# airl-iisc/MRFP

Hardware: AMD Instinct MI355X
Metric: train images/sec (higher is better)
Workload: dtype bf16; 1 GPU; resnet-101 DeepLabV3+ + MRFP+ (HRFP+NP+ on, HRFP re-drawn every step), 768x768, 16 images/GPU, fwd+bwd+SGD, synthetic 19-class, random-init weights; global_batch=16, parallelism=dp1

## Files before the change

include/mrfp_hip.h:

```cpp
#ifndef MRFP_HIP_H
#define MRFP_HIP_H

#include <stdint.h>

#ifdef __cplusplus
extern "C" {
#endif

typedef enum { MRFP_F32 = 0, MRFP_BF16 = 1, MRFP_F16 = 2 } mrfp_dtype;

int mrfp_version(void);
const char* mrfp_last_error(void);

int64_t mrfp_stats_nslab(int64_t B, int64_t Ho);

int mrfp_stats_fwd(const void* x, int dtype, int64_t B, int64_t Ho, int64_t Wo, int64_t C,
                   int64_t Hs, int64_t Ws, const int32_t* tabH, const int32_t* tabW,
                   float* ws, void* stream);

int mrfp_stats_bwd(const void* dy, const void* x, const void* y, const float* mean,
                   const float* fA, const float* fS, int per_image, int dtype, int64_t B, int64_t Ho, int64_t Wo, int64_t C,
                   int64_t Hs, int64_t Ws, const int32_t* tabH, const int32_t* tabW,
                   float* ws, void* stream);
int mrfp_stats_bwd_mask(const void* dy, const void* x, const void* mask, const float* mean, int per_image, int dtype, int64_t B,
// ... 160 lines not shown
                    int dtype, int64_t B, int64_t HW, int64_t C, int64_t ignore_index, int per_image, void* stream);
int mrfp_upsample_region_fwd(const void* P, int64_t ld, const int64_t* target, int dtype, int64_t B, int64_t Hi, int64_t Wi,
                             int64_t H, int64_t W, int64_t C, int64_t ignore_index, const float* weight, int kind, float smooth,
                             int present_only, int per_image, float* ws, float* out, void* stream);
int mrfp_upsample_region_bwd(const void* P, int64_t ld, const int64_t* target, const float* out, const float* gscale,
                             void* dlogits, int64_t Cd, int dtype, int64_t B, int64_t Hi, int64_t Wi, int64_t H, int64_t W,
                             int64_t C, int64_t ignore_index, int per_image, void* stream);

int64_t mrfp_sort_tile_items(void);
int64_t mrfp_sort_scan_sweep(void);
int64_t mrfp_sort_pairs_ws_bytes(int64_t n, int64_t S);
int mrfp_sort_pairs(const void* keys_in, const void* payload_in, void* keys_out, void* payload_out, int64_t n,
                    const int64_t* offsets, int64_t S, int bits, void* ws, void* stream);

int64_t mrfp_lovasz_group_classes(void);
int64_t mrfp_lovasz_ws_bytes(int64_t B, int64_t HW, int64_t C, int per_image);
int64_t mrfp_lovasz_out_floats(int64_t B, int64_t HW, int64_t C, int per_image);
int mrfp_lovasz_fwd(const void* logits, const int64_t* target, int dtype, int64_t B, int64_t HW, int64_t C,
                    int64_t ignore_index, int all_classes, int per_image, void* ws, float* out, void* stream);
int mrfp_lovasz_bwd(const void* logits, const int64_t* target, const float* out, const float* gscale, void* dlogits,
                    int dtype, int64_t B, int64_t HW, int64_t C, int64_t ignore_index, int per_image, void* stream);
int mrfp_upsample_lovasz_fwd(const void* P, int64_t ld, const int64_t* target, int dtype, int64_t B, int64_t Hi, int64_t Wi,
                             int64_t H, int64_t W, int64_t C, int64_t ignore_index, int all_classes, int per_image, void* ws,
                             float* out, void* stream);
int mrfp_upsample_lovasz_bwd(const void* P, int64_t ld, const int64_t* target, const float* out, const float* gscale,
                             void* dlogits, int64_t Cd, int dtype, int64_t B, int64_t Hi, int64_t Wi, int64_t H, int64_t W,
                             int64_t C, int64_t ignore_index, int per_image, void* stream);
int mrfp_lovasz_errors(const void* scores, int64_t ld, const int64_t* target, int dtype, int64_t B, int64_t Hi, int64_t Wi,
                       int64_t H, int64_t W, int64_t C, int64_t ignore_index, float* errors, void* stream);

int mrfp_argmax_hist(const void* logits, const int64_t* target, int dtype, int64_t npix, int64_t C,
                     int64_t* hist, uint8_t* pred, void* stream);

int mrfp_pack_weight(const float* w, void* wf, void* wd, int dtype, int64_t N, int64_t C, int64_t R, int64_t S,
                     int64_t Npad, int64_t Cpad, void* stream);
int mrfp_pack_weights_batched(const void* jobs, const int64_t* prefix, int64_t njobs, int64_t total, int dtype, void* stream);
int mrfp_conv_fwd(const void* x, const void* wpack, const float* bias, void* y, int dtype,
                  int64_t B, int64_t H, int64_t W, int64_t C, int64_t N, int64_t ldy, int64_t R, int64_t S,
                  int64_t Ho, int64_t Wo, int64_t stride, int64_t pad_h, int64_t pad_w, int64_t dil,
                  int64_t sstride, const void* addend, float* colstats, void* stream);
int mrfp_conv_fwd_act(const void* x, const void* wpack, const float* bias, void* y, int dtype,
                      int64_t B, int64_t H, int64_t W, int64_t C, int64_t N, int64_t ldy, int64_t R, int64_t S,
                      int64_t Ho, int64_t Wo, int64_t stride, int64_t pad_h, int64_t pad_w, int64_t dil,
                      int64_t sstride, const void* addend, int act, void* stream);
int mrfp_pack_weight_folded(const float* w, void* wf, const float* conv_bias, const float* bn_weight, const float* bn_bias,
                            const float* running_mean, const float* running_var, float eps, float* bias_out, int dtype,
                            int64_t N, int64_t C, int64_t R, int64_t S, int64_t Npad, int64_t Cpad, void* stream);
int mrfp_pack_weights_folded_batched(const void* jobs, const int64_t* prefix, int64_t njobs, int64_t total, int dtype, void* stream);
int mrfp_conv_stats_layout(int dtype, int64_t B, int64_t H, int64_t W, int64_t C, int64_t N, int64_t ldy, int64_t R, int64_t S,
                           int64_t Ho, int64_t Wo, int64_t stride, int64_t pad_h, int64_t pad_w, int64_t dil, int64_t sstride, int wstats,
                           int64_t* out);
int64_t mrfp_conv_stats_block_rows(int dtype, int64_t B, int64_t H, int64_t W, int64_t C, int64_t N, int64_t R, int64_t S, int64_t Ho,
                                   int64_t Wo, int64_t stride, int64_t pad_h, int64_t pad_w, int64_t dil, int64_t sstride);
int mrfp_conv_single_launch(int64_t B, int64_t image_bytes);
int mrfp_conv_fwd_wstats(const void* x, const void* wpack, const float* bias, void* y, int dtype,
                         int64_t B, int64_t H, int64_t W, int64_t C, int64_t N, int64_t ldy, int64_t R, int64_t S,
                         int64_t Ho, int64_t Wo, int64_t stride, int64_t pad_h, int64_t pad_w, int64_t dil,
                         const uint8_t* rowweight, float* colstats, void* stream);
int mrfp_conv_fwd_gated(const void* x, const void* wpack, const float* bias, void* y, int dtype,
                        int64_t B, int64_t H, int64_t W, int64_t C, int64_t N, int64_t ldy, int64_t R, int64_t S,
                        int64_t Ho, int64_t Wo, int64_t stride, int64_t pad_h, int64_t pad_w, int64_t dil,
                        int64_t sstride, const void* addend, const void* addend_mask, void* stream);
int mrfp_conv_fwd_lowrank(const void* x, const void* wpack, const float* bias, void* y, int dtype,
                          int64_t B, int64_t H, int64_t W, int64_t C, int64_t N, int64_t ldy, int64_t R, int64_t S,
                          int64_t Ho, int64_t Wo, int64_t stride, int64_t pad_h, int64_t pad_w, int64_t dil,
                          int64_t sstride, const void* addend, float* colstats, const void* lr_x, const void* lr_w, int64_t lr_k,
                          void* stream);
int mrfp_conv_lowrank_ok(int dtype, int64_t B, int64_t H, int64_t W, int64_t C, int64_t N, int64_t ldy, int64_t R, int64_t S,
                         int64_t Ho, int64_t Wo, int64_t stride, int64_t pad_h, int64_t pad_w, int64_t dil);
int mrfp_debug_clock_stamps(int family, uint64_t* out, int64_t n);
int64_t mrfp_conv_wgrad_ws_bytes(int64_t M, int64_t N, int64_t Q);
int mrfp_conv_wgrad(const void* x, const void* dy, float* dw, void* ws, int dtype,
                    int64_t B, int64_t H, int64_t W, int64_t C, int64_t Ctrue, int64_t N, int64_t ldn,
                    int64_t R, int64_t S, int64_t Ho, int64_t Wo, int64_t stride, int64_t pad_h, int64_t pad_w,
                    int64_t dil, void* stream);
int64_t mrfp_conv_wgrad_group_max(void);
int64_t mrfp_conv_wgrad_grouped_ws_bytes(int64_t M, int64_t N, int64_t Q, int64_t count);
int mrfp_conv_wgrad_plan(int dtype, int64_t B, int64_t H, int64_t W, int64_t C, int64_t N, int64_t ldn, int64_t R, int64_t S, int64_t Ho,
                         int64_t Wo, int64_t stride, int64_t pad_h, int64_t pad_w, int64_t dil, int64_t count, int64_t* out);
int mrfp_conv_wgrad_grouped(const void* const* xs, const void* const* dys, float* const* dws, int64_t count, void* ws, int dtype,
                            int64_t B, int64_t H, int64_t W, int64_t C, int64_t Ctrue, int64_t N, int64_t ldn,
                            int64_t R, int64_t S, int64_t Ho, int64_t Wo, int64_t stride, int64_t pad_h, int64_t pad_w,
                            int64_t dil, void* stream);
int mrfp_nchw_to_nhwc_pad(const float* x, void* y, int dtype, int64_t B, int64_t C, int64_t H, int64_t W,
                          int64_t Cpad, void* stream);

int mrfp_sgd_step(float* p, const float* g, float* m, int64_t n, float lr, float momentum,
                  float weight_decay, float gscale, int first, void* stream);

int mrfp_grad_accumulate(float* acc, const float* g, int64_t n, int first, void* stream);

int64_t mrfp_grad_check_nblocks(int64_t n);
int mrfp_grad_check(const float* g, int64_t n, float gscale, void* ws, void* state, int dynamic, float growth,
                    float backoff, int growth_interval, float max_norm, void* stream);
int mrfp_sgd_step_checked(float* p, const float* g, float* m, int64_t n, float lr, float momentum,
                          float weight_decay, const void* state, void* stream);

int mrfp_sgd_step_avg(float* p, const float* g, float* m, float* e, int64_t n, float lr, float momentum,
                      float weight_decay, float gscale, int first, int kind, double decay, int warmup, int start,
                      int every, int t, void* stream);
int mrfp_sgd_step_checked_avg(float* p, const float* g, float* m, float* e, int64_t n, float lr, float momentum,
                              float weight_decay, const void* state, int taken_base, int kind, double decay, int warmup,
                              int start, int every, void* stream);
int mrfp_arena_swap(float* a, float* b, int64_t n, void* stream);

int64_t mrfp_group_moments_ws_bytes(int64_t B, int64_t HW, int64_t C);
// ... 82 lines not shown
```

mrfp_amd/csrc/conv_c64.hip:

```cpp
#include "conv_common.hpp"

namespace mrfp {


struct C64P {
    const char* x;
    const char* w;
    char* y;
    const float* bias;
    const char* addend;
    float* colstats;
    const unsigned char* rowweight;
    int B, H, W, N, ldy, dil;
    int strips;
    int units;
    int spi;
    unsigned xbytes, wbytes, ybytes;
    const char* lr_x;
    const char* lr_w;
    unsigned lrbytes;
};

constexpr int kC64Slots = 4;

template <typename T, int CB, int NCG, bool STATS, bool ADD, int ACT = 0, bool LR = false>
__global__ __launch_bounds__(256, (CB == 1 ? 2 : 1)) void conv3x3_c64_kernel(C64P p) {
    static_assert(!LR || (!STATS && !ADD && ACT == 0), "the low-rank operand excludes statistics, an addend and an activation");
    constexpr int PSN = 4 / NCG;
    constexpr int SW = 64 * PSN;
    constexpr int NPIECE = (SW + 4 + 7) / 8;
    constexpr int NPC = CB * NPIECE;
    constexpr int PWV = (NPC + 3) / 4;
    constexpr int SLOT = NPC * 1024;
    constexpr int KS = 18 * CB;
    constexpr int PIXB = 128 * CB;
    constexpr int ST = 4;
    extern __shared__ __attribute__((aligned(16))) char smem[];
    const int t = threadIdx.x, lane = t & 63;
    const int wave = __builtin_amdgcn_readfirstlane(t >> 6);
    const int l15 = lane & 15, lq = lane >> 4;
    const int cg = wave % NCG, ps = wave / NCG;
    const int n0 = (int)blockIdx.y * 128 + cg * 32, nl = n0 + 8 * lq;
    const int d = p.dil;
    const unsigned lds0 = (unsigned)(size_t)(__attribute__((address_space(3))) char*)smem;
    const i32x4 xw = rsrc_words(p.x, p.xbytes);
    const __amdgpu_buffer_rsrc_t wr = __builtin_amdgcn_make_buffer_rsrc((void*)p.w, 0, (int)p.wbytes, 0x00020000);
    const __amdgpu_buffer_rsrc_t yr = __builtin_amdgcn_make_buffer_rsrc((void*)p.y, 0, (int)p.ybytes, 0x00020000);
    const __amdgpu_buffer_rsrc_t ar = __builtin_amdgcn_make_buffer_rsrc((void*)(p.addend ? p.addend : p.y), 0, (int)p.ybytes, 0x00020000);

    uint4 fw[KS][2];
#pragma unroll
    for (int ks = 0; ks < KS; ++ks)
#pragma unroll
        for (int j = 0; j < 2; ++j) {
            const int n = n0 + 8 * (l15 >> 2) + 4 * j + (l15 & 3);
            fw[ks][j] = bload(wr, n < p.N ? (unsigned)n * (unsigned)(1152 * CB) + (unsigned)(ks * 64 + lq * 16) : kOOB);
        }
#pragma unroll
    for (int ks = 0; ks < KS; ++ks)
#pragma unroll
        for (int j = 0; j < 2; ++j) settle(fw[ks][j]);
    const __amdgpu_buffer_rsrc_t lxr = __builtin_amdgcn_make_buffer_rsrc((void*)p.lr_x, 0, (int)p.lrbytes, 0x00020000);
    uint4 fl[2];
    if constexpr (LR) {
        const __amdgpu_buffer_rsrc_t lwr = __builtin_amdgcn_make_buffer_rsrc((void*)p.lr_w, 0, p.N * 64, 0x00020000);
#pragma unroll
        for (int j = 0; j < 2; ++j) {
            const int n = n0 + 8 * (l15 >> 2) + 4 * j + (l15 & 3);
            fl[j] = bload(lwr, n < p.N ? (unsigned)(n * 64 + lq * 16) : kOOB);
        }
#pragma unroll
        for (int j = 0; j < 2; ++j) settle(fl[j]);
    }
    float bv[2][4];
#pragma unroll
    for (int j = 0; j < 2; ++j)
#pragma unroll
        for (int e = 0; e < 4; ++e) bv[j][e] = (p.bias && nl + 4 * j + e < p.N) ? p.bias[nl + 4 * j + e] : 0.f;

    unsigned foff[3][2];
#pragma unroll
    for (int s = 0; s < 3; ++s) {
        const int px = ps * 64 + l15 + s * d;
#pragma unroll
        for (int kk = 0; kk < 2; ++kk) foff[s][kk] = (unsigned)(px * 128 + ((((kk * 4 + lq) ^ px) & 7) << 4));
    }

    float cs[8], cq[8];
#pragma unroll
    for (int u = 0; u < 8; ++u) { cs[u] = 0.f; cq[u] = 0.f; }

    const long long G = gridDim.x;
    int u = (int)((long long)blockIdx.x * p.units / G);
    const int u1 = (int)((long long)(blockIdx.x + 1) * p.units / G);
    const int Hc0 = (p.H + d - 1) / d;
    const int upi = p.strips * p.H;
    int cur_b = -1;
    auto flush = [&](int b) {
        const long long lo = (long long)b * upi, hi = lo + upi;
        int wf = (int)(lo * G / p.units);
        while ((long long)(wf + 1) * p.units / G <= lo) ++wf;
        while (wf > 0 && (long long)wf * p.units / G > lo) --wf;
        const int slot = (int)blockIdx.x - wf;
        float* out = p.colstats + ((size_t)(b * PSN + ps) * p.spi + slot) * 2 * p.ldy;
#pragma unroll
        for (int k = 0; k < 8; ++k) {
            cs[k] = row16_sum(cs[k]);
            cq[k] = row16_sum(cq[k]);
        }
        if (l15 == 0 && nl < p.N) {
#pragma unroll
            for (int k = 0; k < 8; ++k) {
                out[nl + k] = cs[k];
                out[p.ldy + nl + k] = cq[k];
            }
            if ((long long)u1 >= hi) {
                for (int z = slot + 1; z < p.spi; ++z) {
                    float* oz = p.colstats + ((size_t)(b * PSN + ps) * p.spi + z) * 2 * p.ldy;
#pragma unroll
                    for (int k = 0; k < 8; ++k) {
                        oz[nl + k] = 0.f;
                        oz[p.ldy + nl + k] = 0.f;
                    }
                }
            }
        }
#pragma unroll
        for (int k = 0; k < 8; ++k) { cs[k] = 0.f; cq[k] = 0.f; }
    };
    while (u < u1) {
        const int blk_id = u / p.H, tt = u - blk_id * p.H;
        const int b = blk_id / p.strips, strip = blk_id - b * p.strips;
        const int q = (d == 2 && tt >= Hc0) ? 1 : 0;
        const int i0 = tt - q * Hc0;
        const int Hc = q ? p.H - Hc0 : Hc0;
        int i1 = i0 + (u1 - u);
        if (i1 > Hc) i1 = Hc;
        const int ow0 = strip * SW;
        if constexpr (STATS) {
            if (b != cur_b) {
                if (cur_b >= 0) flush(cur_b);
                cur_b = b;
            }
        }
        const unsigned imgbase = (unsigned)b * (unsigned)p.H * (unsigned)p.W * (unsigned)PIXB;
        const int col0 = ow0 - d + (lane >> 3);
        auto issue_row = [&](int i) {
            const int ih = q + d * i;
            const bool rok = i >= 0 && ih < p.H;
            const unsigned rbase = imgbase + (unsigned)(rok ? ih : 0) * (unsigned)p.W * (unsigned)PIXB;
            const unsigned sbase = lds0 + (unsigned)(((i + 4) & 3) * SLOT);
#pragma unroll
            for (int j = 0; j < PWV; ++j) {
                const int pi = j * 4 + wave;
                if (pi >= NPC) continue;
                const int hf = pi / NPIECE, pp = pi - hf * NPIECE;
                const int col = col0 + 8 * pp, px = 8 * pp + (lane >> 3);
                const bool cok = col >= 0 && col < p.W;
                const unsigned cb = (unsigned)(col * PIXB + hf * 128 + (((lane & 7) ^ (px & 7)) << 4));
                dma16_async(xw, sbase + (unsigned)(pi * 1024), (rok && cok) ? rbase + cb : kOOB);
            }
        };
        issue_row(i0 - 1);
        issue_row(i0);
        issue_row(i0 + 1);
        for (int i = i0; i < i1; ++i) {
            if (i == i0) dma_wait<0>();
            else dma_wait<ST>();
            __builtin_amdgcn_s_barrier();
            if (i + 1 < i1) issue_row(i + 2);
            const int oh = q + d * i;
            uint4 av[4];
            unsigned wt[4];
            const int owl = ow0 + ps * 64 + l15;
            const unsigned ml = (unsigned)((b * p.H + oh) * p.W + owl);
            auto out_off = [&](int bk) {
                return (owl + bk * 16 < p.W && nl < p.N) ? ((ml + (unsigned)(bk * 16)) * (unsigned)p.ldy + (unsigned)nl) * 2u : kOOB;
            };
#pragma unroll
            for (int bk = 0; bk < 4; ++bk) {
                if constexpr (ADD) av[bk] = bload(ar, out_off(bk));
                if constexpr (LR) av[bk] = bload(lxr, owl + bk * 16 < p.W ? (ml + (unsigned)(bk * 16)) * 64u + (unsigned)(lq * 16) : kOOB);
                if constexpr (STATS) {
                    const bool ok = owl + bk * 16 < p.W;
                    wt[bk] = ok ? (p.rowweight ? (unsigned)p.rowweight[ml + bk * 16] : 1u) : 0u;
                }
            }
            f32x4 acc[4][2];
            const unsigned sb[3] = {lds0 + (unsigned)(((i + 3) & 3) * SLOT), lds0 + (unsigned)((i & 3) * SLOT),
                                    lds0 + (unsigned)(((i + 1) & 3) * SLOT)};
            uint4 fx[2][4];
            auto read_x = [&](int ks, uint4 (&f)[4]) {
                const int r = ks / (6 * CB), s = (ks / (2 * CB)) % 3, hf = (ks >> 1) % CB, kk = ks & 1;
                const char* base = smem + (sb[r] - lds0) + hf * (NPIECE * 1024) + foff[s][kk];
#pragma unroll
                for (int bk = 0; bk < 4; ++bk) f[bk] = *reinterpret_cast<const uint4*>(base + bk * 2048);
            };
            read_x(0, fx[0]);
#pragma unroll
            for (int ks = 0; ks < KS; ++ks) {
                if (ks + 1 < KS) read_x(ks + 1, fx[(ks + 1) & 1]);
                __builtin_amdgcn_sched_barrier(0);
#pragma unroll
                for (int bk = 0; bk < 4; ++bk)
#pragma unroll
                    for (int j = 0; j < 2; ++j) {
                        if (ks == 0) {
                            const f32x4 z = {bv[j][0], bv[j][1], bv[j][2], bv[j][3]};
                            acc[bk][j] = z;
                        }
                        Mma16<T>::run(acc[bk][j], fw[ks][j], fx[ks & 1][bk]);
                    }
                __builtin_amdgcn_sched_barrier(0);
            }
            if constexpr (LR) {
#pragma unroll
                for (int bk = 0; bk < 4; ++bk) {
                    f32x4 t0 = {0.f, 0.f, 0.f, 0.f}, t1 = {0.f, 0.f, 0.f, 0.f};
                    Mma16<T>::run(t0, fl[0], av[bk]);
                    Mma16<T>::run(t1, fl[1], av[bk]);
                    av[bk] = make_uint4(pack2<T>(t0[0], t0[1]), pack2<T>(t0[2], t0[3]), pack2<T>(t1[0], t1[1]), pack2<T>(t1[2], t1[3]));
                }
            }
#pragma unroll
            for (int bk = 0; bk < 4; ++bk) {
                uint4 v;
                if constexpr (ADD || LR) {
                    float a[8];
                    unpack2<T>(av[bk].x, a[0], a[1]);
                    unpack2<T>(av[bk].y, a[2], a[3]);
                    unpack2<T>(av[bk].z, a[4], a[5]);
                    unpack2<T>(av[bk].w, a[6], a[7]);
                    v.x = pack2<T>(act_f<ACT>(acc[bk][0][0] + a[0]), act_f<ACT>(acc[bk][0][1] + a[1]));
                    v.y = pack2<T>(act_f<ACT>(acc[bk][0][2] + a[2]), act_f<ACT>(acc[bk][0][3] + a[3]));
                    v.z = pack2<T>(act_f<ACT>(acc[bk][1][0] + a[4]), act_f<ACT>(acc[bk][1][1] + a[5]));
                    v.w = pack2<T>(act_f<ACT>(acc[bk][1][2] + a[6]), act_f<ACT>(acc[bk][1][3] + a[7]));
                } else {
                    v.x = pack2<T>(act_f<ACT>(acc[bk][0][0]), act_f<ACT>(acc[bk][0][1]));
                    v.y = pack2<T>(act_f<ACT>(acc[bk][0][2]), act_f<ACT>(acc[bk][0][3]));
                    v.z = pack2<T>(act_f<ACT>(acc[bk][1][0]), act_f<ACT>(acc[bk][1][1]));
                    v.w = pack2<T>(act_f<ACT>(acc[bk][1][2]), act_f<ACT>(acc[bk][1][3]));
                }
                if constexpr (STATS) {
                    float f[8];
                    unpack2<T>(v.x, f[0], f[1]);
                    unpack2<T>(v.y, f[2], f[3]);
                    unpack2<T>(v.z, f[4], f[5]);
                    unpack2<T>(v.w, f[6], f[7]);
                    const float wb = (float)wt[bk];
#pragma unroll
                    for (int k = 0; k < 8; ++k) {
                        const float wf = f[k] * wb;
                        cs[k] += wf;
                        cq[k] += wf * f[k];
                    }
                }
                u32x4 dv;
                dv.x = v.x; dv.y = v.y; dv.z = v.z; dv.w = v.w;
                __builtin_amdgcn_raw_buffer_store_b128(dv, yr, (int)out_off(bk), 0, 0);
            }
        }
        u += i1 - i0;
        asm volatile("s_waitcnt lgkmcnt(0)" ::: "memory");
        __builtin_amdgcn_s_barrier();
    }
    if constexpr (STATS) {
        if (cur_b >= 0) flush(cur_b);
    }
}

static bool c64_applicable(const ConvP& p, int esz) {
    static const int on = env_switch("MRFP_CONV_C64", 1);
    if (!on || esz != 2) return false;
    if (p.R != 3 || p.S != 3 || p.stride != 1 || p.sstride != 1 || p.Ho != p.H || p.Wo != p.W) return false;
    if (p.dil < 1 || p.dil > 2 || p.pad_h != p.dil || p.pad_w != p.dil) return false;
    if ((p.ldy & 7) != 0) return false;
    if (p.C == 64) { if (p.N != 64 && p.N != 128) return false; }
    else if (p.C == 128) {
        static const int c128 = env_switch("MRFP_CONV_C128", 1);
        if (!c128 || (p.N != 64 && p.N != 128 && p.N != 256)) return false;
        const int SW = p.N == 64 ? 128 : 64;
        if (c128 < 2 && (int64_t)p.B * ((p.W + SW - 1) / SW) * p.H < 32 * kGrid1PerCU) return false;
    } else return false;
    if (p.addend_mask || (p.colstats && p.addend)) return false;
    if ((int64_t)p.M * p.ldy * esz >= (int64_t)kOOB || p.H < 2 * p.dil) return false;
    return true;
}
bool c64_plan(const ConvP& p, int esz, ConvPlan& plan) {
    if (!c64_applicable(p, esz)) return false;
    const int SW = p.N == 64 ? 128 : 64;
    const int64_t upi = (int64_t)((p.W + SW - 1) / SW) * p.H, units = upi * p.B;
    const int64_t cap = p.C == 64 ? kGrid2PerCU : kGrid1PerCU;
    plan.kind = ConvKernel::c64;
    plan.tile_rows = 0;
    plan.grid = (int)(units < cap ? units : cap);
    plan.spi = (int)(upi / (units / plan.grid) + 2);
    const int64_t rows_per_image = (int64_t)(p.N == 64 ? 2 : 1) * plan.spi;
    plan.stats_blocks = p.B * rows_per_image;
    plan.stats_block_rows = -rows_per_image;
    return true;
}

template <typename T, int CB, int NCG, bool STATS, bool ADD, int ACT = 0, bool LR = false>
static int c64_launch(const C64P& q, int grid, hipStream_t st) {
    constexpr int SW = 64 * (4 / NCG), NPIECE = (SW + 4 + 7) / 8;
    const int lds = kC64Slots * CB * NPIECE * 1024 + 1024;
    static bool attr_set = false;
    if (!attr_set) {
        (void)hipFuncSetAttribute(reinterpret_cast<const void*>(&conv3x3_c64_kernel<T, CB, NCG, STATS, ADD, ACT, LR>),
                                  hipFuncAttributeMaxDynamicSharedMemorySize, lds);
        attr_set = true;
    }
    hipLaunchKernelGGL((conv3x3_c64_kernel<T, CB, NCG, STATS, ADD, ACT, LR>), dim3((unsigned)grid, (unsigned)((q.N + 127) / 128)), dim3(256), lds, st, q);
    MRFP_LAUNCH_CHECK();
    return 0;
}
template <typename T, int CB, int NCG>
static int c64_pick(const ConvP& p, const C64P& q, int grid, hipStream_t st, int act) {
    if (q.lr_x) {
        MRFP_CHECK(act == 0 && !p.colstats && !p.addend, "conv_fwd_lowrank: no activation, statistics or addend beside the low-rank operand");
        return c64_launch<T, CB, NCG, false, false, 0, true>(q, grid, st);
    }
    if (act != 0) {
        if (p.colstats) return -1;
        if (act == 1) return p.addend ? c64_launch<T, CB, NCG, false, true, 1>(q, grid, st) : c64_launch<T, CB, NCG, false, false, 1>(q, grid, st);
        return p.addend ? c64_launch<T, CB, NCG, false, true, 2>(q, grid, st) : c64_launch<T, CB, NCG, false, false, 2>(q, grid, st);
    }
    if (p.colstats) return c64_launch<T, CB, NCG, true, false>(q, grid, st);
    if (p.addend) return c64_launch<T, CB, NCG, false, true>(q, grid, st);
    return c64_launch<T, CB, NCG, false, false>(q, grid, st);
}

template <typename T>
static int c64_run_t(const ConvP& p, const ConvPlan& plan, hipStream_t st, int act, const void* lr_x, const void* lr_w) {
    C64P q;
    q.lr_x = (const char*)lr_x; q.lr_w = (const char*)lr_w; q.lrbytes = lr_x ? (unsigned)((int64_t)p.M * 64) : 0u;
    q.x = p.x; q.w = p.w; q.y = p.y; q.bias = p.bias; q.addend = p.addend; q.colstats = p.colstats; q.rowweight = p.rowweight;
    q.B = p.B; q.H = p.H; q.W = p.W; q.N = p.N; q.ldy = p.ldy; q.dil = p.dil;
    const int SW = p.N == 64 ? 128 : 64;
    q.strips = (p.W + SW - 1) / SW;
    q.units = p.B * q.strips * p.H;
    q.spi = plan.spi;
    q.xbytes = p.xbytes; q.wbytes = p.wbytes; q.ybytes = (unsigned)((int64_t)p.M * p.ldy * 2);
    const int grid = plan.grid;
    if (p.C == 64) return p.N == 64 ? c64_pick<T, 1, 2>(p, q, grid, st, act) : c64_pick<T, 1, 4>(p, q, grid, st, act);
    return p.N == 64 ? c64_pick<T, 2, 2>(p, q, grid, st, act) : c64_pick<T, 2, 4>(p, q, grid, st, act);
}
int c64_run(const ConvP& p, const ConvPlan& plan, bool is_f16, hipStream_t st, int act, const void* lr_x, const void* lr_w) {
    MRFP_CHECK(!lr_x == !lr_w, "conv_fwd_lowrank: both low-rank operands or neither");
    return is_f16 ? c64_run_t<f16>(p, plan, st, act, lr_x, lr_w) : c64_run_t<bf16>(p, plan, st, act, lr_x, lr_w);
}

}
```

mrfp_amd/csrc/conv_common.hpp:

```cpp
#pragma once
#include "common.hpp"
#include <stdlib.h>

#ifndef MRFP_VMCNT0
#define MRFP_VMCNT0 0
#endif

#ifndef MRFP_CLOCK_STAMP
#define MRFP_CLOCK_STAMP 0
#endif

namespace mrfp {

constexpr int kGrid1PerCU = kCUs;
constexpr int kGrid2PerCU = 2 * kCUs;

constexpr int kStampSlots = 4096;
#if MRFP_CLOCK_STAMP
struct ClockStamp {
    unsigned long long t0, r0;
    __device__ __forceinline__ void begin() {
        t0 = __builtin_amdgcn_s_memtime();
        r0 = __builtin_amdgcn_s_memrealtime();
        __builtin_amdgcn_s_waitcnt(0xC07F);
// ... 189 lines not shown
    unsigned short h;
    __builtin_memcpy(&h, &x, 2);
    const unsigned sh = (u & 1) ? 16u : 0u, mask = ~(0xffffu << sh), bits = (unsigned)h << sh;
    if ((u >> 1) == 0) v.x = (v.x & mask) | bits;
    else if ((u >> 1) == 1) v.y = (v.y & mask) | bits;
    else if ((u >> 1) == 2) v.z = (v.z & mask) | bits;
    else v.w = (v.w & mask) | bits;
}
template <typename T> __device__ __forceinline__ uint4 chunk_add(const uint4& a, const uint4& b) {
    uint4 r = make_uint4(0u, 0u, 0u, 0u);
#pragma unroll
    for (int u = 0; u < 16 / (int)sizeof(T); ++u) chunk_set<T>(r, u, from_f<T>(to_f(chunk_get<T>(a, u)) + to_f(chunk_get<T>(b, u))));
    return r;
}

template <typename T, int ACT> __device__ __forceinline__ uint4 chunk_act(const uint4& a) {
    uint4 r = make_uint4(0u, 0u, 0u, 0u);
#pragma unroll
    for (int u = 0; u < 16 / (int)sizeof(T); ++u) chunk_set<T>(r, u, from_f<T>(act_f<ACT>(to_f(chunk_get<T>(a, u)))));
    return r;
}

#ifndef MRFP_RR_HOLD
#define MRFP_RR_HOLD 1
#endif
__device__ __forceinline__ uint4 gate_chunk16(const uint4& v, unsigned bits) {
    auto w = [&](unsigned word, int u) {
        const unsigned keep = (((bits >> u) & 1u) ? 0x0000ffffu : 0u) | (((bits >> (u + 1)) & 1u) ? 0xffff0000u : 0u);
        return word & keep;
    };
    return make_uint4(w(v.x, 0), w(v.y, 2), w(v.z, 4), w(v.w, 6));
}

#ifndef MRFP_EARLY_FULL
#define MRFP_EARLY_FULL 1
#endif

enum class ConvKernel { pw, pwk, c64, rr384, rr192, t256x64, t192x128, t96x128, t128x128 };
struct ConvPlan {
    ConvKernel kind;
    int tile_rows;
    int64_t stats_blocks;
    int64_t stats_block_rows;
    int grid, spi;
};

bool pw_plan(const ConvP& p, int esz, ConvPlan& plan);
int pw_run(const ConvP& p, bool is_f16, hipStream_t st, int act = 0);

bool pwk_plan(const ConvP& p, int esz, ConvPlan& plan);
int pwk_run(const ConvP& p, bool is_f16, hipStream_t st, int act = 0);

bool c64_plan(const ConvP& p, int esz, ConvPlan& plan);
int c64_run(const ConvP& p, const ConvPlan& plan, bool is_f16, hipStream_t st, int act = 0, const void* lr_x = nullptr,
            const void* lr_w = nullptr);

constexpr int kWgMaxGroup = 32;
struct WgGroup {
    const char* x[kWgMaxGroup];
    const char* dy[kWgMaxGroup];
};
inline WgGroup make_wg_group(const void* const* xs, const void* const* dys, int64_t count) {
    WgGroup g;
    for (int i = 0; i < kWgMaxGroup; ++i) {
        g.x[i] = (const char*)xs[i < count ? i : 0];
        g.dy[i] = (const char*)dys[i < count ? i : 0];
    }
    return g;
}

struct ClassWalk {
    int Wp, a, L, R, Wr, splits;
};
inline bool class_walk(int64_t ncls, int64_t U, int per_round, int64_t count, ClassWalk& w) {
    w.Wp = (int)(per_round / count);
    if (ncls * U < w.Wp) w.Wp = (int)(ncls * U);
    w.a = (int)(w.Wp / ncls);
    if (w.a < 1) return false;
    w.L = (int)((ncls * U + w.Wp - 1) / w.Wp);
    const int64_t main = (int64_t)w.a * w.L < U ? (int64_t)w.a * w.L : U;
    w.R = (int)(U - main);
    w.Wr = (int)(w.Wp - w.a * ncls);
    if (w.R > 0 && w.Wr == 0) return false;
    w.splits = w.a + (w.R > 0 ? 2 : 0);
    return true;
}
inline int64_t class_walk_slots(int64_t ncls, int per_round, int64_t count) {
    const int64_t a = (per_round / count) / ncls;
    return a < 1 ? 0 : a + 2;
}
struct WgradGeom {
    int esz;
    int64_t B, H, W, C, N, ldn, R, S, Ho, Wo, stride, pad_h, pad_w, dil, count;
    int64_t M() const { return B * Ho * Wo; }
    int64_t Q() const { return R * S * C; }
    bool pointwise() const { return R == 1 && S == 1 && stride == 1 && pad_h == 0 && pad_w == 0 && H == Ho && W == Wo; }
};
enum class WgradKernel { wg3, wg1, t64x256, t128x128, t256x128 };
enum { kWgDma = 1, kWgDense = 2 };
struct WgradPlan {
    WgradKernel kind;
    int variant;
    int splits;
    int klen;
    int grid;
    int tiles;
// ... 15 lines not shown
```

mrfp_amd/csrc/conv_igemm.hip:

```cpp
#include "conv_common.hpp"
#include <type_traits>

namespace mrfp {

MRFP_STAMP_DECL(g_stamps_igemm)
int stamps_igemm(unsigned long long* out, int n) { return MRFP_STAMP_READ(g_stamps_igemm, out, n); }

template <typename T, int WM, int WN, bool ALIGNED, bool STRIDED, int TM, int TN, bool RR = false, int ACT = 0>
__global__ __launch_bounds__(64 * WM * WN, ((RR && TM * TN >= 6) ? 2 : 3)) void conv_igemm_kernel(ConvP p) {
    constexpr int NT = 64 * WM * WN, BM = 32 * TM * WM, BN = 32 * TN * WN;
    constexpr int SA = BM * 8 / NT, SB = BN * 8 / NT, RSTEP = NT / 8;
    extern __shared__ __attribute__((aligned(16))) char smem[];
    char* const sA0 = smem;
    char* const sB0 = smem + BM * 128;
    MRFP_STAMP_BEGIN();

    const int t = threadIdx.x, lane = t & 63, wave = t >> 6;
    const int wm = wave / WN, wn = wave % WN;
    const int ntn = (p.N + BN - 1) / BN;
    const int tile = xcd_remap(blockIdx.x, gridDim.x);
    const int m0 = (tile / ntn) * BM, n0 = (tile % ntn) * BN;
    const int rbase = t >> 3;
    const int chunk = (t & 7) ^ ((rbase >> 1) & 7);
    const int wrow = __builtin_amdgcn_readfirstlane(wave) * 8;
// ... 757 lines not shown

int mrfp_conv_fwd_gated(const void* x, const void* wpack, const float* bias, void* y, int dtype, int64_t B, int64_t H,
                        int64_t W, int64_t C, int64_t N, int64_t ldy, int64_t R, int64_t S, int64_t Ho, int64_t Wo,
                        int64_t stride, int64_t pad_h, int64_t pad_w, int64_t dil, int64_t sstride, const void* addend,
                        const void* addend_mask, void* stream) {
    MRFP_CHECK(addend && addend_mask, "conv_fwd_gated: addend and its gate mask are required");
    return conv_fwd_impl(x, wpack, bias, y, dtype, B, H, W, C, N, ldy, R, S, Ho, Wo, stride, pad_h, pad_w, dil, sstride, addend,
                         nullptr, stream, addend_mask);
}

int mrfp_conv_fwd_lowrank(const void* x, const void* wpack, const float* bias, void* y, int dtype, int64_t B, int64_t H,
                          int64_t W, int64_t C, int64_t N, int64_t ldy, int64_t R, int64_t S, int64_t Ho, int64_t Wo,
                          int64_t stride, int64_t pad_h, int64_t pad_w, int64_t dil, int64_t sstride, const void* addend,
                          float* colstats, const void* lr_x, const void* lr_w, int64_t lr_k, void* stream) {
    MRFP_CHECK(!addend && !colstats, "conv_fwd_lowrank: the low-rank operand excludes an addend and statistics");
    MRFP_CHECK(lr_x && lr_w && aligned16(lr_x) && aligned16(lr_w), "conv_fwd_lowrank: both low-rank operands are required, 16-byte aligned");
    MRFP_CHECK(lr_k == 32, "conv_fwd_lowrank: the low-rank K is 32, got %lld", (long long)lr_k);
    MRFP_CHECK(dtype == MRFP_BF16 || dtype == MRFP_F16, "conv_fwd_lowrank: 16-bit activations only (dtype %d)", dtype);
    return conv_fwd_impl(x, wpack, bias, y, dtype, B, H, W, C, N, ldy, R, S, Ho, Wo, stride, pad_h, pad_w, dil, sstride, nullptr,
                         nullptr, stream, nullptr, nullptr, 0, lr_x, lr_w);
}

int mrfp_conv_lowrank_ok(int dtype, int64_t B, int64_t H, int64_t W, int64_t C, int64_t N, int64_t ldy, int64_t R, int64_t S,
                         int64_t Ho, int64_t Wo, int64_t stride, int64_t pad_h, int64_t pad_w, int64_t dil) {
    if (!dtype_known(dtype) || dtype_bytes(dtype) != 2) return 0;
    ConvP p;
    if (conv_params(p, dtype, B, H, W, C, N, ldy, R, S, Ho, Wo, stride, pad_h, pad_w, dil, 1, nullptr, nullptr, nullptr, nullptr, nullptr))
        return 0;
    if (!mrfp_conv_single_launch(B, H * W * C * 2)) return 0;
    return conv_plan(p, 2).kind == ConvKernel::c64 ? 1 : 0;
}

int mrfp_conv_stats_layout(int dtype, int64_t B, int64_t H, int64_t W, int64_t C, int64_t N, int64_t ldy, int64_t R, int64_t S,
                           int64_t Ho, int64_t Wo, int64_t stride, int64_t pad_h, int64_t pad_w, int64_t dil, int64_t sstride, int wstats,
                           int64_t* out) {
    MRFP_CHECK(out, "conv_stats_layout: no output array");
    float stats_present;
    unsigned char rows_present;
    ConvP p;
    const int bad = conv_params(p, dtype, B, H, W, C, N, ldy, R, S, Ho, Wo, stride, pad_h, pad_w, dil, sstride, nullptr, nullptr,
                                nullptr, &stats_present, wstats ? &rows_present : nullptr);
    if (bad) return bad;
    const ConvPlan plan = conv_plan(p, dtype_bytes(dtype));
    const int64_t nblk = plan.stats_blocks;
    const bool compact = nblk > kCompactAbove;
    out[0] = nblk;
    out[1] = plan.stats_block_rows;
    out[2] = compact ? nblk + kStatGroups : nblk;
    out[3] = compact ? nblk : 0;
    out[4] = compact ? kStatGroups : nblk;
    return 0;
}

int64_t mrfp_conv_stats_block_rows(int dtype, int64_t B, int64_t H, int64_t W, int64_t C, int64_t N, int64_t R, int64_t S, int64_t Ho,
                                   int64_t Wo, int64_t stride, int64_t pad_h, int64_t pad_w, int64_t dil, int64_t sstride) {
    int64_t lay[5];
    return mrfp_conv_stats_layout(dtype, B, H, W, C, N, N, R, S, Ho, Wo, stride, pad_h, pad_w, dil, sstride, 0, lay) ? 0 : lay[1];
}


}
```

Baseline: 305.8 images/sec.

## Specialize c64 conv row loop by valid column blocks and cost-balance work split

For the CB==2 c64 3x3 conv kernel, the per-row compute body moves into an included header and is instantiated for 0-4 valid 16-column blocks. Partial edge strips then skip MFMA, LDS reads and stores for out-of-range columns. The work split across workgroups is weighted by per-unit cost, with edge strips cheaper, so blocks stay balanced, and the stats-slot lookup is updated to match. A debug API exposes the span layout. Risks are more code variants, register and compile cost, and DMA wait counts now tied to NB.

After: 302.4 images/sec. -1.1%, worse.

```diff
diff --git a/include/mrfp_hip.h b/include/mrfp_hip.h
--- a/include/mrfp_hip.h
+++ b/include/mrfp_hip.h
@@ -236,6 +236,7 @@
                            int64_t* out);
 int64_t mrfp_conv_stats_block_rows(int dtype, int64_t B, int64_t H, int64_t W, int64_t C, int64_t N, int64_t R, int64_t S, int64_t Ho,
                                    int64_t Wo, int64_t stride, int64_t pad_h, int64_t pad_w, int64_t dil, int64_t sstride);
+int64_t mrfp_conv_c64_spans(int dtype, int64_t B, int64_t H, int64_t W, int64_t C, int64_t N, int64_t dil, int64_t* out, int64_t n);
 int mrfp_conv_single_launch(int64_t B, int64_t image_bytes);
 int mrfp_conv_fwd_wstats(const void* x, const void* wpack, const float* bias, void* y, int dtype,
                          int64_t B, int64_t H, int64_t W, int64_t C, int64_t N, int64_t ldy, int64_t R, int64_t S,
diff --git a/mrfp_amd/csrc/conv_c64.hip b/mrfp_amd/csrc/conv_c64.hip
--- a/mrfp_amd/csrc/conv_c64.hip
+++ b/mrfp_amd/csrc/conv_c64.hip
@@ -19,9 +19,45 @@
     const char* lr_x;
     const char* lr_w;
     unsigned lrbytes;
+    int cl;
+    int bycost;
 };
 
 constexpr int kC64Slots = 4;
+
+#ifndef MRFP_C64_EDGES
+#define MRFP_C64_EDGES 1
+#endif
+constexpr bool kC64Edges(int CB) { return MRFP_C64_EDGES && CB == 2; }
+
+struct C64Split {
+    int B, H, strips, units, cl, bycost;
+    long long G;
+    __host__ __device__ long long upi() const { return (long long)strips * H; }
+    __host__ __device__ long long image_cost() const { return (long long)H * (4 * (strips - 1) + cl); }
+    __host__ __device__ int start(long long g) const {
+        if (!bycost) return (int)(g * units / G);
+        const long long CI = image_cost(), T = g * (CI * B) / G, b = T / CI, r = T - b * CI, full = 4LL * (strips - 1) * H;
+        if (b >= B) return units;
+        return (int)(b * upi() + (r < full ? (r + 2) / 4 : (long long)(strips - 1) * H + (r - full + cl / 2) / cl));
+    }
+    __host__ __device__ int first_wg(int b) const {
+        const long long lo = (long long)b * upi();
+        int wf = (int)((long long)b * G / B);
+        while (start(wf + 1) <= lo) ++wf;
+        while (wf > 0 && start(wf) > lo) --wf;
+        return wf;
+    }
+};
+static C64Split c64_split(int B, int H, int W, int C, int N, long long G) {
+    C64Split s;
+    const int SW = N == 64 ? 128 : 64;
+    s.B = B; s.H = H; s.strips = (W + SW - 1) / SW; s.units = B * s.strips * H; s.G = G;
+    const int last = (W - (s.strips - 1) * SW + 15) / 16;
+    s.cl = kC64Edges(C / 64) ? (last < 4 ? last : 4) : 4;
+    s.bycost = s.cl < 4 && s.strips > 1 && s.image_cost() * B / G >= 4;
+    return s;
+}
 
 template <typename T, int CB, int NCG, bool STATS, bool ADD, int ACT = 0, bool LR = false>
 __global__ __launch_bounds__(256, (CB == 1 ? 2 : 1)) void conv3x3_c64_kernel(C64P p) {
@@ -34,7 +70,6 @@
     constexpr int SLOT = NPC * 1024;
     constexpr int KS = 18 * CB;
     constexpr int PIXB = 128 * CB;
-    constexpr int ST = 4;
     extern __shared__ __attribute__((aligned(16))) char smem[];
     const int t = threadIdx.x, lane = t & 63;
     const int wave = __builtin_amdgcn_readfirstlane(t >> 6);
@@ -91,16 +126,22 @@
     for (int u = 0; u < 8; ++u) { cs[u] = 0.f; cq[u] = 0.f; }
 
     const long long G = gridDim.x;
-    int u = (int)((long long)blockIdx.x * p.units / G);
-    const int u1 = (int)((long long)(blockIdx.x + 1) * p.units / G);
+    C64Split sp;
+    sp.B = p.B; sp.H = p.H; sp.strips = p.strips; sp.units = p.units; sp.cl = p.cl; sp.bycost = p.bycost; sp.G = G;
+    int u = kC64Edges(CB) ? sp.start(blockIdx.x) : (int)((long long)blockIdx.x * p.units / G);
+    const int u1 = kC64Edges(CB) ? sp.start((long long)blockIdx.x + 1) : (int)((long long)(blockIdx.x + 1) * p.units / G);
     const int Hc0 = (p.H + d - 1) / d;
     const int upi = p.strips * p.H;
     int cur_b = -1;
     auto flush = [&](int b) {
         const long long lo = (long long)b * upi, hi = lo + upi;
-        int wf = (int)(lo * G / p.units);
-        while ((long long)(wf + 1) * p.units / G <= lo) ++wf;
-        while (wf > 0 && (long long)wf * p.units / G > lo) --wf;
+        int wf;
+        if constexpr (kC64Edges(CB)) wf = sp.first_wg(b);
+        else {
+            wf = (int)(lo * G / p.units);
+            while ((long long)(wf + 1) * p.units / G <= lo) ++wf;
+            while (wf > 0 && (long long)wf * p.units / G > lo) --wf;
+        }
         const int slot = (int)blockIdx.x - wf;
         float* out = p.colstats + ((size_t)(b * PSN + ps) * p.spi + slot) * 2 * p.ldy;
 #pragma unroll
@@ -164,102 +205,33 @@
         issue_row(i0 - 1);
         issue_row(i0);
         issue_row(i0 + 1);
-        for (int i = i0; i < i1; ++i) {
-            if (i == i0) dma_wait<0>();
-            else dma_wait<ST>();
-            __builtin_amdgcn_s_barrier();
-            if (i + 1 < i1) issue_row(i + 2);
-            const int oh = q + d * i;
-            uint4 av[4];
-            unsigned wt[4];
-            const int owl = ow0 + ps * 64 + l15;
-            const unsigned ml = (unsigned)((b * p.H + oh) * p.W + owl);
-            auto out_off = [&](int bk) {
-                return (owl + bk * 16 < p.W && nl < p.N) ? ((ml + (unsigned)(bk * 16)) * (unsigned)p.ldy + (unsigned)nl) * 2u : kOOB;
-            };
-#pragma unroll
-            for (int bk = 0; bk < 4; ++bk) {
-                if constexpr (ADD) av[bk] = bload(ar, out_off(bk));
-                if constexpr (LR) av[bk] = bload(lxr, owl + bk * 16 < p.W ? (ml + (unsigned)(bk * 16)) * 64u + (unsigned)(lq * 16) : kOOB);
-                if constexpr (STATS) {
-                    const bool ok = owl + bk * 16 < p.W;
-                    wt[bk] = ok ? (p.rowweight ? (unsigned)p.rowweight[ml + bk * 16] : 1u) : 0u;
+#define C64_ROWS(nb) { constexpr int NB = nb, NBA = NB ? NB : 1; (void)NBA;
+        if constexpr (kC64Edges(CB)) {
+            int nb = (p.W - ow0 - ps * 64 + 15) >> 4;
+            nb = nb < 0 ? 0 : nb > 4 ? 4 : nb;
+            switch (nb) {
+            case 4: C64_ROWS(4)
+#include "conv_c64_rows.hpp"
+                } break;
+            case 3: C64_ROWS(3)
+#include "conv_c64_rows.hpp"
+                } break;
+            case 2: C64_ROWS(2)
+#include "conv_c64_rows.hpp"
+                } break;
+            case 1: C64_ROWS(1)
+#include "conv_c64_rows.hpp"
+                } break;
+            default:
+                if constexpr (PSN > 1) C64_ROWS(0)
+#include "conv_c64_rows.hpp"
                 }
-            }
-            f32x4 acc[4][2];
-            const unsigned sb[3] = {lds0 + (unsigned)(((i + 3) & 3) * SLOT), lds0 + (unsigned)((i & 3) * SLOT),
-                                    lds0 + (unsigned)(((i + 1) & 3) * SLOT)};
-            uint4 fx[2][4];
-            auto read_x = [&](int ks, uint4 (&f)[4]) {
-                const int r = ks / (6 * CB), s = (ks / (2 * CB)) % 3, hf = (ks >> 1) % CB, kk = ks & 1;
-                const char* base = smem + (sb[r] - lds0) + hf * (NPIECE * 1024) + foff[s][kk];
-#pragma unroll
-                for (int bk = 0; bk < 4; ++bk) f[bk] = *reinterpret_cast<const uint4*>(base + bk * 2048);
-            };
-            read_x(0, fx[0]);
-#pragma unroll
-            for (int ks = 0; ks < KS; ++ks) {
-                if (ks + 1 < KS) read_x(ks + 1, fx[(ks + 1) & 1]);
-                __builtin_amdgcn_sched_barrier(0);
-#pragma unroll
-                for (int bk = 0; bk < 4; ++bk)
-#pragma unroll
-                    for (int j = 0; j < 2; ++j) {
-                        if (ks == 0) {
-                            const f32x4 z = {bv[j][0], bv[j][1], bv[j][2], bv[j][3]};
-                            acc[bk][j] = z;
-                        }
-                        Mma16<T>::run(acc[bk][j], fw[ks][j], fx[ks & 1][bk]);
-                    }
-                __builtin_amdgcn_sched_barrier(0);
-            }
-            if constexpr (LR) {
-#pragma unroll
-                for (int bk = 0; bk < 4; ++bk) {
-                    f32x4 t0 = {0.f, 0.f, 0.f, 0.f}, t1 = {0.f, 0.f, 0.f, 0.f};
-                    Mma16<T>::run(t0, fl[0], av[bk]);
-                    Mma16<T>::run(t1, fl[1], av[bk]);
-                    av[bk] = make_uint4(pack2<T>(t0[0], t0[1]), pack2<T>(t0[2], t0[3]), pack2<T>(t1[0], t1[1]), pack2<T>(t1[2], t1[3]));
-                }
-            }
-#pragma unroll
-            for (int bk = 0; bk < 4; ++bk) {
-                uint4 v;
-                if constexpr (ADD || LR) {
-                    float a[8];
-                    unpack2<T>(av[bk].x, a[0], a[1]);
-                    unpack2<T>(av[bk].y, a[2], a[3]);
-                    unpack2<T>(av[bk].z, a[4], a[5]);
-                    unpack2<T>(av[bk].w, a[6], a[7]);
-                    v.x = pack2<T>(act_f<ACT>(acc[bk][0][0] + a[0]), act_f<ACT>(acc[bk][0][1] + a[1]));
-                    v.y = pack2<T>(act_f<ACT>(acc[bk][0][2] + a[2]), act_f<ACT>(acc[bk][0][3] + a[3]));
-                    v.z = pack2<T>(act_f<ACT>(acc[bk][1][0] + a[4]), act_f<ACT>(acc[bk][1][1] + a[5]));
-                    v.w = pack2<T>(act_f<ACT>(acc[bk][1][2] + a[6]), act_f<ACT>(acc[bk][1][3] + a[7]));
-                } else {
-                    v.x = pack2<T>(act_f<ACT>(acc[bk][0][0]), act_f<ACT>(acc[bk][0][1]));
-                    v.y = pack2<T>(act_f<ACT>(acc[bk][0][2]), act_f<ACT>(acc[bk][0][3]));
-                    v.z = pack2<T>(act_f<ACT>(acc[bk][1][0]), act_f<ACT>(acc[bk][1][1]));
-                    v.w = pack2<T>(act_f<ACT>(acc[bk][1][2]), act_f<ACT>(acc[bk][1][3]));
-                }
-                if constexpr (STATS) {
-                    float f[8];
-                    unpack2<T>(v.x, f[0], f[1]);
-                    unpack2<T>(v.y, f[2], f[3]);
-                    unpack2<T>(v.z, f[4], f[5]);
-                    unpack2<T>(v.w, f[6], f[7]);
-                    const float wb = (float)wt[bk];
-#pragma unroll
-                    for (int k = 0; k < 8; ++k) {
-                        const float wf = f[k] * wb;
-                        cs[k] += wf;
-                        cq[k] += wf * f[k];
-                    }
-                }
-                u32x4 dv;
-                dv.x = v.x; dv.y = v.y; dv.z = v.z; dv.w = v.w;
-                __builtin_amdgcn_raw_buffer_store_b128(dv, yr, (int)out_off(bk), 0, 0);
-            }
-        }
+                break;
+            }
+        } else C64_ROWS(4)
+#include "conv_c64_rows.hpp"
+        }
+#undef C64_ROWS
         u += i1 - i0;
         asm volatile("s_waitcnt lgkmcnt(0)" ::: "memory");
         __builtin_amdgcn_s_barrier();
@@ -301,6 +273,17 @@
     return true;
 }
 
+int64_t c64_spans(const ConvP& p, const ConvPlan& plan, int64_t* out, int64_t n) {
+    const C64Split sp = c64_split(p.B, p.H, p.W, p.C, p.N, plan.grid);
+    const int64_t G = plan.grid, need = 6 + G + p.B;
+    if (!out) return G;
+    if (n < need) return -need;
+    out[0] = sp.units; out[1] = sp.upi(); out[2] = plan.spi; out[3] = sp.cl; out[4] = sp.bycost;
+    for (int64_t g = 0; g <= G; ++g) out[5 + g] = sp.start(g);
+    for (int b = 0; b < p.B; ++b) out[6 + G + b] = sp.first_wg(b);
+    return G;
+}
+
 template <typename T, int CB, int NCG, bool STATS, bool ADD, int ACT = 0, bool LR = false>
 static int c64_launch(const C64P& q, int grid, hipStream_t st) {
     constexpr int SW = 64 * (4 / NCG), NPIECE = (SW + 4 + 7) / 8;
@@ -341,6 +324,8 @@
     q.strips = (p.W + SW - 1) / SW;
     q.units = p.B * q.strips * p.H;
     q.spi = plan.spi;
+    const C64Split sp = c64_split(p.B, p.H, p.W, p.C, p.N, plan.grid);
+    q.cl = sp.cl; q.bycost = sp.bycost;
     q.xbytes = p.xbytes; q.wbytes = p.wbytes; q.ybytes = (unsigned)((int64_t)p.M * p.ldy * 2);
     const int grid = plan.grid;
     if (p.C == 64) return p.N == 64 ? c64_pick<T, 1, 2>(p, q, grid, st, act) : c64_pick<T, 1, 4>(p, q, grid, st, act);
diff --git a/mrfp_amd/csrc/conv_c64_rows.hpp b/mrfp_amd/csrc/conv_c64_rows.hpp
--- /dev/null
+++ b/mrfp_amd/csrc/conv_c64_rows.hpp
@@ -0,0 +1,97 @@
+        for (int i = i0; i < i1; ++i) {
+            if (i == i0) dma_wait<0>();
+            else dma_wait<NB>();
+            __builtin_amdgcn_s_barrier();
+            if (i + 1 < i1) issue_row(i + 2);
+            if constexpr (NB == 0) continue;
+            const int oh = q + d * i;
+            uint4 av[NBA];
+            unsigned wt[NBA];
+            const int owl = ow0 + ps * 64 + l15;
+            const unsigned ml = (unsigned)((b * p.H + oh) * p.W + owl);
+            auto out_off = [&](int bk) {
+                return (owl + bk * 16 < p.W && nl < p.N) ? ((ml + (unsigned)(bk * 16)) * (unsigned)p.ldy + (unsigned)nl) * 2u : kOOB;
+            };
+#pragma unroll
+            for (int bk = 0; bk < NB; ++bk) {
+                if constexpr (ADD) av[bk] = bload(ar, out_off(bk));
+                if constexpr (LR) av[bk] = bload(lxr, owl + bk * 16 < p.W ? (ml + (unsigned)(bk * 16)) * 64u + (unsigned)(lq * 16) : kOOB);
+                if constexpr (STATS) {
+                    const bool ok = owl + bk * 16 < p.W;
+                    wt[bk] = ok ? (p.rowweight ? (unsigned)p.rowweight[ml + bk * 16] : 1u) : 0u;
+                }
+            }
+            f32x4 acc[NBA][2];
+            const unsigned sb[3] = {lds0 + (unsigned)(((i + 3) & 3) * SLOT), lds0 + (unsigned)((i & 3) * SLOT),
+                                    lds0 + (unsigned)(((i + 1) & 3) * SLOT)};
+            uint4 fx[2][NBA];
+            auto read_x = [&](int ks, uint4 (&f)[NBA]) {
+                const int r = ks / (6 * CB), s = (ks / (2 * CB)) % 3, hf = (ks >> 1) % CB, kk = ks & 1;
+                const char* base = smem + (sb[r] - lds0) + hf * (NPIECE * 1024) + foff[s][kk];
+#pragma unroll
+                for (int bk = 0; bk < NB; ++bk) f[bk] = *reinterpret_cast<const uint4*>(base + bk * 2048);
+            };
+            read_x(0, fx[0]);
+#pragma unroll
+            for (int ks = 0; ks < KS; ++ks) {
+                if (ks + 1 < KS) read_x(ks + 1, fx[(ks + 1) & 1]);
+                __builtin_amdgcn_sched_barrier(0);
+#pragma unroll
+                for (int bk = 0; bk < NB; ++bk)
+#pragma unroll
+                    for (int j = 0; j < 2; ++j) {
+                        if (ks == 0) {
+                            const f32x4 z = {bv[j][0], bv[j][1], bv[j][2], bv[j][3]};
+                            acc[bk][j] = z;
+                        }
+                        Mma16<T>::run(acc[bk][j], fw[ks][j], fx[ks & 1][bk]);
+                    }
+                __builtin_amdgcn_sched_barrier(0);
+            }
+            if constexpr (LR) {
+#pragma unroll
+                for (int bk = 0; bk < NB; ++bk) {
+                    f32x4 t0 = {0.f, 0.f, 0.f, 0.f}, t1 = {0.f, 0.f, 0.f, 0.f};
+                    Mma16<T>::run(t0, fl[0], av[bk]);
+                    Mma16<T>::run(t1, fl[1], av[bk]);
+                    av[bk] = make_uint4(pack2<T>(t0[0], t0[1]), pack2<T>(t0[2], t0[3]), pack2<T>(t1[0], t1[1]), pack2<T>(t1[2], t1[3]));
+                }
+            }
+#pragma unroll
+            for (int bk = 0; bk < NB; ++bk) {
+                uint4 v;
+                if constexpr (ADD || LR) {
+                    float a[8];
+                    unpack2<T>(av[bk].x, a[0], a[1]);
+                    unpack2<T>(av[bk].y, a[2], a[3]);
+                    unpack2<T>(av[bk].z, a[4], a[5]);
+                    unpack2<T>(av[bk].w, a[6], a[7]);
+                    v.x = pack2<T>(act_f<ACT>(acc[bk][0][0] + a[0]), act_f<ACT>(acc[bk][0][1] + a[1]));
+                    v.y = pack2<T>(act_f<ACT>(acc[bk][0][2] + a[2]), act_f<ACT>(acc[bk][0][3] + a[3]));
+                    v.z = pack2<T>(act_f<ACT>(acc[bk][1][0] + a[4]), act_f<ACT>(acc[bk][1][1] + a[5]));
+                    v.w = pack2<T>(act_f<ACT>(acc[bk][1][2] + a[6]), act_f<ACT>(acc[bk][1][3] + a[7]));
+                } else {
+                    v.x = pack2<T>(act_f<ACT>(acc[bk][0][0]), act_f<ACT>(acc[bk][0][1]));
+                    v.y = pack2<T>(act_f<ACT>(acc[bk][0][2]), act_f<ACT>(acc[bk][0][3]));
+                    v.z = pack2<T>(act_f<ACT>(acc[bk][1][0]), act_f<ACT>(acc[bk][1][1]));
+                    v.w = pack2<T>(act_f<ACT>(acc[bk][1][2]), act_f<ACT>(acc[bk][1][3]));
+                }
+                if constexpr (STATS) {
+                    float f[8];
+                    unpack2<T>(v.x, f[0], f[1]);
+                    unpack2<T>(v.y, f[2], f[3]);
+                    unpack2<T>(v.z, f[4], f[5]);
+                    unpack2<T>(v.w, f[6], f[7]);
+                    const float wb = (float)wt[bk];
+#pragma unroll
+                    for (int k = 0; k < 8; ++k) {
+                        const float wf = f[k] * wb;
+                        cs[k] += wf;
+                        cq[k] += wf * f[k];
+                    }
+                }
+                u32x4 dv;
+                dv.x = v.x; dv.y = v.y; dv.z = v.z; dv.w = v.w;
+                __builtin_amdgcn_raw_buffer_store_b128(dv, yr, (int)out_off(bk), 0, 0);
+            }
+        }
diff --git a/mrfp_amd/csrc/conv_common.hpp b/mrfp_amd/csrc/conv_common.hpp
--- a/mrfp_amd/csrc/conv_common.hpp
+++ b/mrfp_amd/csrc/conv_common.hpp
@@ -265,6 +265,7 @@
 int pwk_run(const ConvP& p, bool is_f16, hipStream_t st, int act = 0);
 
 bool c64_plan(const ConvP& p, int esz, ConvPlan& plan);
+int64_t c64_spans(const ConvP& p, const ConvPlan& plan, int64_t* out, int64_t n);
 int c64_run(const ConvP& p, const ConvPlan& plan, bool is_f16, hipStream_t st, int act = 0, const void* lr_x = nullptr,
             const void* lr_w = nullptr);
 
diff --git a/mrfp_amd/csrc/conv_igemm.hip b/mrfp_amd/csrc/conv_igemm.hip
--- a/mrfp_amd/csrc/conv_igemm.hip
+++ b/mrfp_amd/csrc/conv_igemm.hip
@@ -833,6 +833,14 @@
     return 0;
 }
 
+int64_t mrfp_conv_c64_spans(int dtype, int64_t B, int64_t H, int64_t W, int64_t C, int64_t N, int64_t dil, int64_t* out, int64_t n) {
+    ConvP p;
+    if (conv_params(p, dtype, B, H, W, C, N, N, 3, 3, H, W, 1, dil, dil, dil, 1, nullptr, nullptr, nullptr, nullptr, nullptr)) return -1;
+    const ConvPlan plan = conv_plan(p, dtype_bytes(dtype));
+    if (plan.kind != ConvKernel::c64) return 0;
+    return c64_spans(p, plan, out, n);
+}
+
 int64_t mrfp_conv_stats_block_rows(int dtype, int64_t B, int64_t H, int64_t W, int64_t C, int64_t N, int64_t R, int64_t S, int64_t Ho,
                                    int64_t Wo, int64_t stride, int64_t pad_h, int64_t pad_w, int64_t dil, int64_t sstride) {
     int64_t lay[5];
```
